# AIBluefisher/DAGSfM

Measured on AMD Instinct MI355X. Metric: verified image-pairs/sec (+ RANSAC hypotheses/sec) at 4096 feats/image, higher is better.
Workload: dtype u8 matching (int8 MFMA) + f64 verification

## Files before the change

### dagsfm_amd/capi.py

```python
import ctypes
import os

import numpy as np

_HERE = os.path.dirname(os.path.abspath(__file__))
LIB_PATH = os.environ.get("DSM_LIB_PATH") or os.path.join(_HERE, "libdagsfm_mi355x.so")
CHECK_LIB_PATH = os.environ.get("DSM_CHECK_LIB_PATH") or os.path.join(_HERE, "libdagsfm_mi355x_check.so")

GATHER_LIB_PATH = os.path.join(_HERE, "libdagsfm_gather.so")

u8p = ctypes.POINTER(ctypes.c_uint8)
u32p = ctypes.POINTER(ctypes.c_uint32)
u64p = ctypes.POINTER(ctypes.c_uint64)
f32p = ctypes.POINTER(ctypes.c_float)


class DsmError(RuntimeError):
    pass


class MatchOptions(ctypes.Structure):
    _fields_ = [("max_ratio", ctypes.c_double), ("max_distance", ctypes.c_double),
                ("cross_check", ctypes.c_int32), ("max_num_matches", ctypes.c_int32)]

# ... 1007 lines not shown
            "track_offsets": np.concatenate([[0], np.cumsum([len(t) for t in tracks])]).astype(np.uint32),
            "obs_image": np.array([img_new[int(oimg[k])] for t in tracks for k in t], np.uint32),
            "obs_xy": (np.concatenate([oxy[t] for t in tracks]) if tracks else np.zeros((0, 2))).reshape(-1, 2),
            "image_index": np.array(images, np.int64), "camera_index": np.array(cams, np.int64),
            "point_index": np.array(points, np.int64)}


def absolute_pose_seed(problem, factor_index, user_seed=0):
    return int(lib().dsm_absolute_pose_seed(problem, factor_index, user_seed))


def absolute_pose_factors(options=None):
    o = options if options is not None else default_absolute_pose_options()
    n = int(lib().dsm_absolute_pose_factors(ctypes.byref(o), None, 0))
    out = np.zeros(max(n, 1))
    lib().dsm_absolute_pose_factors(ctypes.byref(o), out.ctypes.data, n)
    return out[:n].copy()


def absolute_pose_max_trials(options=None):
    o = options if options is not None else default_absolute_pose_options()
    return int(lib().dsm_absolute_pose_max_trials(ctypes.byref(o)))


def align_seed(i, j, direction, user_seed=0):
    return int(lib().dsm_align_seed(i, j, direction, user_seed))


PRODUCT_OPTION_KEYS = ("DSM_MATCH_CHUNK_ROWS", "DSM_VERIFY_CHUNK_PAIRS", "DSM_VERIFY_LANES", "DSM_VERIFY_INLINE_LO", "DSM_VERIFY_ITEM_MODE",
                       "DSM_LO_TAIL", "DSM_LO_TAIL_MODE", "DSM_VERIFY_GRID_DIV")
CHECK_OPTION_KEYS = ("DSM_K1_DOT4", "DSM_K1_RESOLVE_KERNEL", "DSM_VERIFY_DEBUG", "DSM_SAMPLER_SERIAL", "DSM_LO_PREPARE_WAVE", "DSM_LO_JACOBI_GROUPS", "DSM_ROOTS_LDS",
                     "DSM_FINAL_WAVES", "DSM_VERIFY_LEGACY", "DSM_VERIFY_FIXED_BATCH", "DSM_VERIFY_LANE_SPLIT", "DSM_DEBUG_SAMPLER_MODE",
                     "DSM_VOCAB_ASSIGN_VALU", "DSM_VERIFY_HOST_LOOP", "DSM_SCORE_PREFILTER", "DSM_VERIFY_REPLAY_GRID", "DSM_REPLAY_LEGACY", "DSM_FLANN_GROUP", "DSM_FLANN_STATS", "DSM_ELU_LDS", "DSM_HYP_GRID", "DSM_SPEC_MARGIN",
                     "DSM_POSE_FULL", "DSM_PATCH_MATCH_LANES", "DSM_NORMS_EXACT", "DSM_FUSION_SERIAL")
DEBUG_OPTION_KEYS = PRODUCT_OPTION_KEYS


def check_requested():
    return os.environ.get("DSM_LIBRARY") == "check" or any(os.environ.get(k) is not None for k in CHECK_OPTION_KEYS)


class Context:

    def __init__(self, device=0, check=None):
        self._handle = ctypes.c_void_p()
        self._debug = {}
        self.check = check_requested() if check is None else bool(check)
        self._L = lib(self.check)
        rc = self._L.dsm_ctx_create(device, ctypes.byref(self._handle))
        if rc != 0:
            raise DsmError("dsm_ctx_create failed (%d): %s" % (rc, self._L.dsm_last_error(None).decode()))
        self.n_pairs = 0

    @property
    def _h(self):
        if self._handle:
            for key in PRODUCT_OPTION_KEYS + CHECK_OPTION_KEYS:
                want = os.environ.get(key)
                if self._debug.get(key) != want:
                    self.set_debug_option(key, want)
        return self._handle

    def set_memory_budget(self, nbytes):
        self._L.dsm_ctx_set_memory_budget.argtypes = [ctypes.c_void_p, ctypes.c_uint64]
        self._chk(self._L.dsm_ctx_set_memory_budget(self._handle, ctypes.c_uint64(int(nbytes))))

    def memory_footprint(self):
# ... 1087 lines not shown
```

### dagsfm_amd/csrc/capi.hip

```cpp
#include <hip/hip_runtime.h>
#include <math.h>
#include <stdint.h>
#include <stdio.h>
#include <stdlib.h>
#include <string.h>

#include <algorithm>
#include <string>
#include <system_error>
#include <thread>
#include <vector>

#include "../../include/dagsfm_mi355x.h"
#include "ctx.h"
#include "kernels.h"
#include "verify_camera.h"

namespace {
thread_local std::string g_create_error;
}

static const uint64_t kStageSlot = 16ull << 20;
static const uint64_t kStageSmall = 1ull << 20;
static const unsigned kStageThreads = 8;
// ... 1073 lines not shown
  vp.samples = nullptr;
  vp.draws_end = nullptr;
  vp.nmodels = nullptr;
  vp.counts = nullptr;
  vp.sums = nullptr;
  vp.first_batch[0] = vp.first_batch[1] = vp.first_batch[2] = 0;
  vp.stats = ctx->dbg("DSM_VERIFY_DEBUG") ? 1 : 0;
  vp.norms_exact = ctx->dbg("DSM_NORMS_EXACT") ? 1 : 0;
  vp.lo_reg_prepare = ctx->dbg("DSM_LO_PREPARE_WAVE") ? 0 : 1;
  vp.rp_cap = std::min<uint32_t>(n_max, 256u);
  vp.spec_margin[0] = 8;
  vp.spec_margin[1] = vp.spec_margin[2] = 4;
  if (const char* e = ctx->dbg("DSM_SPEC_MARGIN")) {
    unsigned a = 8, b = 4;
    if (sscanf(e, "%u,%u", &a, &b) == 2) {
      vp.spec_margin[0] = a;
      vp.spec_margin[1] = b;
    }
  }
  vp.hyp_map = nullptr;
  vp.hyp_seg_cap = 0;
  vp.replay_legacy = ctx->dbg("DSM_REPLAY_LEGACY") ? 1 : 0;
  vp.dbg_elu_lds = ctx->dbg("DSM_ELU_LDS") ? 1 : 0;
  vp.dbg_jacobi_groups = ctx->dbg("DSM_LO_JACOBI_GROUPS") ? 1 : 0;
  vp.dbg_roots_lds = ctx->dbg("DSM_ROOTS_LDS") ? 1 : 0;
  vp.dbg_final_waves = ctx->dbg("DSM_FINAL_WAVES") ? atoi(ctx->dbg("DSM_FINAL_WAVES")) : 0;
  vp.dbg_pose_full = ctx->dbg("DSM_POSE_FULL") ? 1 : 0;
  vp.score_prefilter = ctx->dbg("DSM_SCORE_PREFILTER") ? atoi(ctx->dbg("DSM_SCORE_PREFILTER")) : 1;
  const bool prefilter_check = ctx->dbg("DSM_SCORE_PREFILTER") && strcmp(ctx->dbg("DSM_SCORE_PREFILTER"), "check") == 0;
  if (prefilter_check) {
    vp.score_prefilter = 5;
    vp.stats = 1;
  }
  vp.models = nullptr;
  vp.e_work = nullptr;
  vp.sidx_g = nullptr;
  vp.active_count = nullptr;
  vp.lo_inl = nullptr;
  vp.worklist = nullptr;
  vp.n_work = 0;
  vp.lo_queue_g = nullptr;
  vp.lo_queue = nullptr;
  vp.lo_count = nullptr;
  vp.lo_work = vp.lo_models = vp.lo_slots = vp.lo_ework = nullptr;
  vp.tail_items = nullptr;
  vp.tail_n = nullptr;
  vp.lo_jobs = nullptr;
  vp.lo_inl_pool = nullptr;
  vp.job_list = nullptr;
#ifdef DSM_CHECK_BUILD
  const bool legacy = ctx->dbg("DSM_VERIFY_LEGACY") != nullptr;
#else
  const bool legacy = false;
#endif
  if (legacy) {
#ifdef DSM_CHECK_BUILD
    HIPCHK(ctx, ctx->d_vscratch.reserve(std::max<size_t>(1, (size_t)n_blocks * verify_scratch_bytes_per_block(n_max))));
    vp.scratch = ctx->d_vscratch.as<double>();
    HIPCHK(ctx, ctx->lanes[0].active.reserve(LANE_CTR_BYTES));
    HIPCHK(ctx, hipMemsetAsync(ctx->lanes[0].active.p, 0, LANE_CTR_BYTES, st));
    vp.active_count = ctx->lanes[0].active.as<uint32_t>() + LANE_CTR_AREA / 4;
    HIPCHK(ctx, hipEventRecord(ctx->vev0, st));
    launch_verify(vp, n_blocks, st);
    HIPCHK(ctx, hipGetLastError());
#endif
  } else {
// ... 771 lines not shown
```

### dagsfm_amd/csrc/ctx.h

```cpp
#ifndef DAGSFM_AMD_CSRC_CTX_H_
#define DAGSFM_AMD_CSRC_CTX_H_

#include <hip/hip_runtime.h>
#include <stdint.h>

#include <map>
#include <string>
#include <vector>

#include "../../include/dagsfm_mi355x.h"

struct DevBuf {
  void* p = nullptr;
  size_t cap = 0;
  DevBuf() = default;
  DevBuf(const DevBuf&) = delete;
  DevBuf& operator=(const DevBuf&) = delete;
  DevBuf(DevBuf&& o) noexcept : p(o.p), cap(o.cap) {
    o.p = nullptr;
    o.cap = 0;
  }
  DevBuf& operator=(DevBuf&& o) noexcept {
    if (this != &o) {
      release();
// ... 198 lines not shown
  std::vector<double> cluster_ritz, cluster_vectors;
  uint32_t cluster_rows = 0, cluster_cols = 0;

  template <typename F>
  void for_each_buffer(F f) {
    for (DevBuf* b : {&d_desc, &d_rterm, &d_kp, &d_img_row0, &d_img_rows, &d_lut, &d_stage, &d_counts, &d_offsets, &d_matches, &d_total, &d_etotal,
                      &d_cams, &d_pairs_dev, &d_seeds, &d_tvg, &d_inl, &d_inl_counts, &d_inl_off, &d_inl_compact, &d_inl_total, &d_nt_table,
                      &d_nt_off, &d_nt_off_t, &d_pair_state, &d_pts_px, &d_pts_norm, &d_reports, &d_masks, &d_fam_state, &d_sidx, &d_lo_inl,
                      &d_nt_table_t, &d_wm_redo, &d_wm_total, &d_wm_count, &d_lo_inl_pool, &d_pose_jobs,
                      &d_g_nfeat, &d_g_dpairs, &d_g_doff, &d_g_pdir, &d_g_params, &d_g_m, &d_g_counts, &d_g_offsets, &d_g_total, &d_g_matches,
                      &d_g_plan, &d_g_inl, &d_g_inl_off,
                      &d_mm_matches[0], &d_mm_matches[1], &d_mm_off[0], &d_mm_off[1], &d_mm_counts, &d_mm_state, &d_mm_first, &d_mm_acc,
                      &d_mm_keep, &d_mm_total, &d_vb_desc, &d_vb_idx})
      f(*b, false);
    for (DevBuf* b : {&d_m, &d_ms, &d_entries, &d_out2, &d_out2s, &d_dpairs, &d_dpairs2, &d_doutoff, &d_pair_dir, &d_order, &d_ecnt, &d_eoff,
                      &d_runs, &d_run_blocks, &d_run_blkoff, &d_gblocks, &d_egrow,
                      &d_vscratch, &d_ud_border, &d_ud_points, &d_ud_src, &d_ud_dst, &d_ud_map, &d_pm, &d_vb_point, &d_vb_node, &d_vb_embed, &d_sf_maps, &d_sf_lanes})
      f(*b, true);
    for (VerifyLane& L : lanes) L.for_each_buffer([&f](DevBuf& b) { f(b, true); });
  }
};
void dsm_retrieval_destroy(dsm_ctx* ctx);
void dsm_retrieval_invalidate(dsm_ctx* ctx);
void dsm_sift_destroy(dsm_ctx* ctx);
void dsm_covariant_sift_destroy(dsm_ctx* ctx);

static const char* const dsm_product_debug_keys[] = {"DSM_MATCH_CHUNK_ROWS", "DSM_VERIFY_CHUNK_PAIRS", "DSM_VERIFY_LANES", "DSM_VERIFY_INLINE_LO",
                                                     "DSM_VERIFY_ITEM_MODE", "DSM_LO_TAIL", "DSM_LO_TAIL_MODE", "DSM_VERIFY_GRID_DIV"};
#ifdef DSM_CHECK_BUILD
static const char* const dsm_check_debug_keys[] = {"DSM_K1_DOT4", "DSM_K1_RESOLVE_KERNEL", "DSM_VERIFY_DEBUG", "DSM_SAMPLER_SERIAL", "DSM_LO_PREPARE_WAVE", "DSM_LO_JACOBI_GROUPS",
                                                   "DSM_ROOTS_LDS", "DSM_FINAL_WAVES", "DSM_VERIFY_LEGACY", "DSM_VERIFY_FIXED_BATCH", "DSM_VERIFY_LANE_SPLIT",
                                                   "DSM_DEBUG_SAMPLER_MODE", "DSM_VOCAB_ASSIGN_VALU", "DSM_VERIFY_HOST_LOOP", "DSM_SCORE_PREFILTER",
                                                   "DSM_VERIFY_REPLAY_GRID", "DSM_REPLAY_LEGACY", "DSM_FLANN_GROUP", "DSM_FLANN_STATS", "DSM_ELU_LDS", "DSM_HYP_GRID", "DSM_SPEC_MARGIN",
                                                   "DSM_POSE_FULL", "DSM_PATCH_MATCH_LANES", "DSM_NORMS_EXACT", "DSM_FUSION_SERIAL"};
#endif

#define HIPCHK(ctx, call)                                                              \
  do {                                                                                 \
    hipError_t e_ = (call);                                                            \
    if (e_ != hipSuccess) {                                                            \
      (ctx)->err = std::string(#call) + ": " + hipGetErrorString(e_);                  \
      return DSM_ERR_HIP;                                                              \
    }                                                                                  \
  } while (0)

#define HIPTRY(call)                                                   \
  do {                                                                 \
    hipError_t e_ = (call);                                            \
    if (e_ != hipSuccess && rc == DSM_OK) {                            \
      ctx->err = std::string(#call) + ": " + hipGetErrorString(e_);    \
      rc = DSM_ERR_HIP;                                                \
    }                                                                  \
  } while (0)

static inline int dsm_fail(dsm_ctx* ctx, int code, const char* msg) {
  if (ctx) ctx->err = msg;
  return code;
}

#endif
```

### dagsfm_amd/csrc/kernels.h

```cpp
#ifndef DAGSFM_AMD_CSRC_KERNELS_H_
#define DAGSFM_AMD_CSRC_KERNELS_H_

#include <hip/hip_runtime.h>
#include <stdint.h>

#include "../../include/dagsfm_mi355x.h"

struct K1Params {
  const int8_t* desc;
  const int32_t* rterm;
  const uint2* dpairs;
  const uint32_t* img_row0;
  const uint32_t* img_rows;
  const uint64_t* d_out_off;
  const float* lut;
  float max_ratio;
  float max_distance;
  int32_t* out;
  int32_t* out_s;
  const uint32_t* order;
  const uint2* entries;
  const uint64_t* e_off;
  const uint32_t* e_cnt;
  const uint4* gblocks;
// ... 60 lines not shown
  uint32_t m_pos;
  uint32_t lo_wait;
  uint32_t lo_ninl;
  uint32_t lo_nm;
  uint32_t pad;
};
#define LO_WORK_DOUBLES 176

#define TAIL_KMAX 8
struct PoseJob {
  int32_t ncmb;
  int32_t ni;
  double Rc[4 * 9];
  double tc[4 * 3];
  int32_t cnt[4];
  double med[4];
};
struct LoJob {
  uint32_t pl;
  uint32_t ninl;
  uint32_t pending;
  uint32_t nm;
};
struct TailItem {
  uint32_t t, m;
  uint32_t nlo;
  uint32_t out_n;
  double out_sum;
  double out_model[9];
};

#ifndef DSM_REPLAY_WAVES
#define DSM_REPLAY_WAVES 4
#endif

struct VerifyParams {
  const uint32_t* pairs;
  const uint64_t* match_off;
  const uint32_t* matches;
  const double* kp;
  const uint32_t* img_row0;
  const dsm_camera* cams;
  dsm_two_view_options opt;
  const uint32_t* seeds;
  const uint32_t* nt_table;
  const uint64_t* nt_off;
  const uint32_t* nt_table_t;
  const uint64_t* nt_off_t;
  uint32_t* wm_redo;
  uint32_t* wm_total;
  uint32_t* wm_count;
  const uint32_t* final_list;
  PoseJob* pose_jobs;
  uint32_t n_final;
  uint32_t max_trials[4];
  uint32_t first_batch[3];
  dsm_two_view_geometry* tvg;
  uint32_t* inlier_matches;
  uint32_t* inl_counts;
  double* scratch;
  uint32_t* pair_state;
  double* pts_px;
  double* pts_norm;
  RansacReport* reports;
  unsigned char* masks;
  uint64_t mask_stride;
// ... 12 lines not shown
  int norms_exact;
  uint32_t spec_margin[3];
  uint32_t* hyp_map;
  uint32_t hyp_seg_cap;
  uint32_t rp_cap;
  int replay_legacy;
  double* models;
  uint32_t* sidx_g;
  uint32_t* active_count;
  uint32_t pair0, n_chunk;
  uint32_t batch;
  uint32_t n_pairs;
  uint32_t n_max;
  int32_t stage_filter;
  double* e_work;
  int32_t sampler_serial;
  int32_t reseed;
  int32_t keep_generator;
  uint32_t* lo_inl;
  TailItem* tail_items;
  uint32_t* tail_n;
  struct LoJob* lo_jobs;
  uint32_t* lo_inl_pool;
  uint32_t* job_list;
  const uint32_t* worklist;
  uint32_t n_work;
  uint32_t* lo_queue_g;
  uint32_t* lo_queue;
  uint32_t* lo_count;
  double* lo_work;
  double* lo_models;
  double* lo_slots;
  double* lo_ework;
};

size_t verify_scratch_bytes_per_block(uint32_t n_max);
size_t verify_smem_bytes(uint32_t n_max);
void launch_verify(const VerifyParams& p, uint32_t n_blocks, hipStream_t st);
void launch_vp_prep(const VerifyParams& p, uint32_t n_blocks, hipStream_t st);
void launch_vp_sample(const VerifyParams& p, int fam, uint32_t n_blocks, hipStream_t st);
void launch_vp_solve_score(const VerifyParams& p, int fam, hipStream_t st);
void launch_vp_replay(const VerifyParams& p, int fam, uint32_t n_blocks, hipStream_t st);
void launch_vp_final(const VerifyParams& p, uint32_t n_blocks, hipStream_t st);
void launch_vp_replay_lo(const VerifyParams& p, int fam, uint32_t n_blocks, int mode, hipStream_t st);
void launch_vp_items_enum(const VerifyParams& p, int fam, hipStream_t st);
void launch_vp_items_inliers(const VerifyParams& p, int fam, uint32_t n_blocks, hipStream_t st);
void launch_vp_items_outcome(const VerifyParams& p, int fam, uint32_t n_blocks, hipStream_t st);
void launch_vp_local_opt(const VerifyParams& p, int fam, uint32_t n_blocks, uint32_t n_wave_prepare, uint32_t n_small_jacobi, uint32_t n_big_prepare, hipStream_t st);
void launch_lane_counters(const void* src, uint32_t* dst_host, uint32_t copy_bytes, void* zero, size_t zero_bytes, hipStream_t st);
uint32_t vp_batch(int fam, uint32_t max_trials, uint32_t min_trials);
uint32_t vp_maxm(int fam);
void debug_read_prof(unsigned long long* out16);
void launch_debug_samples(uint32_t seed, uint32_t k, uint32_t total, uint32_t n_draws, uint32_t* out, uint32_t* idx, uint32_t* tmp7,
                          int mode, hipStream_t st);
void launch_debug_image_to_world(const dsm_camera& cam, uint32_t n, const double* xy, double* uv, hipStream_t st);
void launch_compact_inliers(const uint64_t* match_off, const uint64_t* inl_off, const uint32_t* inl_counts,
                            const uint32_t* src, uint32_t* dst, uint32_t n_pairs, hipStream_t st);

void launch_k0(const uint8_t* in_u8, int8_t* out_s8, int32_t* rterm, uint64_t n_rows, hipStream_t st);
void launch_k1(const K1Params& p, uint32_t n_directed, uint32_t max_row_blocks, hipStream_t st);
void launch_run_blocks(const uint32_t* run_first, uint32_t n_runs, const uint64_t* e_off, uint32_t* run_blocks, uint64_t* run_blkoff,
                       hipStream_t st);
void launch_gather_blocks(const uint32_t* run_first, uint32_t n_runs, const uint64_t* e_off, const uint2* dpairs, const uint64_t* run_blkoff,
                          uint4* gblocks, uint32_t n_slots, hipStream_t st);
void launch_k1_gather(const K1Params& p, uint32_t n_slots, hipStream_t st);
void launch_k1_dot4(const K1Params& p, uint32_t n_directed, uint32_t max_row_blocks, hipStream_t st);
// ... 41 lines not shown
```

### dagsfm_amd/csrc/verify_kernels.hip

```cpp
#include <hip/hip_runtime.h>
#include <stddef.h>
#include <stdint.h>

#include "../../include/dagsfm_mi355x.h"
#include "kernels.h"
#include "verify_estimators.h"
#include "verify_camera.h"
#include "verify_fivept_coop.h"

#define BATCH 64

struct MtState {
  uint32_t mt[624];
  int mti;
  uint32_t calls;
};

struct VSmem {
  WvSvdShared svd;
  double sv[9];
  double lo_models[90];
  double cur_model[9];
  double bcast[16];
  int ibcast[8];
// ... 2039 lines not shown
  for (int k = 0; k < 9; ++k) M[k] = has_model ? gm[k] : 0.0;
  int lb = 0, sure_out = n + 1;
  if (in_lds) {
    double mx[4];
    stage_points_with_maxima(gpts, n, true, spts, lane, mx);
    if (has_model) {
      const PreBounds b = prescore_bounds<FAM>(M, mx, T);
      sure_out = 0;
#pragma unroll 4
      for (int i = 0; i < n; ++i) prescore_point<FAM>(M, b, spts + (size_t)i * 4, lb, sure_out);
    }
  } else {
    double mx[4];
    stage_points_with_maxima(gpts, n, false, nullptr, lane, mx);
    if (has_model) {
      const PreBounds b = prescore_bounds<FAM>(M, mx, T);
      sure_out = 0;
#pragma unroll 4
      for (int i = 0; i < n; ++i) prescore_point<FAM>(M, b, gpts + (size_t)i * 4, lb, sure_out);
    }
  }
  if (has_slot) {
    p.counts[((size_t)pl * p.batch + t) * F::MAXM + m] = n - sure_out;
    reinterpret_cast<int32_t*>(p.sums + ((size_t)pl * p.batch + t) * F::MAXM + m)[0] = lb;
  }
}

typedef float dsm_f32x2 __attribute__((ext_vector_type(2)));
DSM_DEV dsm_f32x2 pk_fma(dsm_f32x2 a, dsm_f32x2 b, dsm_f32x2 c) { return __builtin_elementwise_fma(a, b, c); }
DSM_DEV dsm_f32x2 pk2(float x) {
  dsm_f32x2 v = {x, x};
  return v;
}
#define PRESCORE_LIST_CAP 24
__global__ __launch_bounds__(64, 6) void k_prescore_h2(const VerifyParams p) {
  extern __shared__ __attribute__((aligned(16))) unsigned char smem_raw[];
  float* s32 = reinterpret_cast<float*>(smem_raw);
  const uint32_t pl = blockIdx.x;
  const uint32_t pi = p.pair0 + pl;
  const FamState* fs = p.fam_state + (size_t)pi * 3 + FAM_H;
  if (!fs->active) return;
  const int lane = threadIdx.x;
  const int nb = (int)fs->nb;
  const int t = blockIdx.y * 64 + lane;
  if ((int)(blockIdx.y * 64) >= nb) return;
  const uint64_t moff = p.match_off[pi];
  const int n = (int)(p.match_off[pi + 1] - moff);
  const double* gpts = p.pts_px + 4 * moff;
  const bool in_lds = n <= VP_LDS_PTS;
  const double T = p.opt.max_error * p.opt.max_error;
  const bool has_slot = t < nb;
  const bool has_model = has_slot && 0 < p.nmodels[(size_t)pl * p.batch + (has_slot ? t : 0)];
  const double* gm = p.models + ((size_t)pl * p.batch + (has_slot ? t : 0)) * 9;
  double M[9];
  for (int k = 0; k < 9; ++k) M[k] = has_model ? gm[k] : 0.0;
  int lb = 0, sure_out = n + 1;
  double mx[4];
  stage_points_with_maxima(gpts, n, false, nullptr, lane, mx);
  if (!in_lds) {
    if (has_model) {
      const PreBounds b = prescore_bounds<FAM_H>(M, mx, T);
      sure_out = 0;
#pragma unroll 4
      for (int i = 0; i < n; ++i) prescore_point<FAM_H>(M, b, gpts + (size_t)i * 4, lb, sure_out);
    }
  } else {
    const int npair = (n + 1) / 2;
    uint16_t* lst = reinterpret_cast<uint16_t*>(s32 + (size_t)8 * npair);
    for (int j = lane; j < npair; j += 64) {
      const int ia = 2 * j, ib = 2 * j + 1 < n ? 2 * j + 1 : 2 * j;
      float4 lo, hi;
      lo.x = (float)gpts[ia * 4 + 0];
      lo.y = (float)gpts[ib * 4 + 0];
      lo.z = (float)gpts[ia * 4 + 1];
      lo.w = (float)gpts[ib * 4 + 1];
      hi.x = (float)gpts[ia * 4 + 2];
      hi.y = (float)gpts[ib * 4 + 2];
      hi.z = (float)gpts[ia * 4 + 3];
      hi.w = (float)gpts[ib * 4 + 3];
      reinterpret_cast<float4*>(s32)[2 * j] = lo;
      reinterpret_cast<float4*>(s32)[2 * j + 1] = hi;
    }
// ... 55 lines not shown
    }
    const bool overflow = cnt > PRESCORE_LIST_CAP;
    if (overflow) {
      lb = 0;
      sure_out = 0;
      for (int i = 0; i < n; ++i) prescore_point<FAM_H>(M, b, gpts + (size_t)i * 4, lb, sure_out);
      cnt = 0;
    }
    int maxc = cnt;
#pragma unroll
    for (int o = 32; o > 0; o >>= 1) maxc = max(maxc, __shfl_xor(maxc, o));
    for (int k0 = 0; k0 < maxc; k0 += 4) {
      double q[4][4];
      bool on[4];
#pragma unroll
      for (int u = 0; u < 4; ++u) {
        on[u] = k0 + u < cnt;
        const double* src = gpts + (size_t)(on[u] ? lst[(k0 + u) * 64 + lane] : 0) * 4;
#pragma unroll
        for (int c = 0; c < 4; ++c) q[u][c] = src[c];
      }
#pragma unroll
      for (int u = 0; u < 4; ++u) {
        bool in, out;
        prescore_flags<FAM_H>(M, b, q[u], in, out);
        lb += (on[u] && in) ? 1 : 0;
        sure_out += (on[u] && out) ? 1 : 0;
      }
    }
  }
  if (has_slot) {
    p.counts[(size_t)pl * p.batch + t] = n - sure_out;
    reinterpret_cast<int32_t*>(p.sums + (size_t)pl * p.batch + t)[0] = lb;
  }
}

#ifdef DSM_CHECK_BUILD
#define PRESCORE_CU_MFMA 0x1p-50
typedef double dsm_f64x4 __attribute__((ext_vector_type(4)));
__global__ __launch_bounds__(64, 4) void k_prescore_h_mfma(const VerifyParams p) {
  extern __shared__ __attribute__((aligned(16))) unsigned char smem_raw[];
  double* spts = reinterpret_cast<double*>(smem_raw);
  const uint32_t pl = blockIdx.x;
  const uint32_t pi = p.pair0 + pl;
  const FamState* fs = p.fam_state + (size_t)pi * 3 + FAM_H;
  if (!fs->active) return;
  const int lane = threadIdx.x;
  const int nb = (int)fs->nb;
  const int t0 = (int)blockIdx.y * 64;
  if (t0 >= nb) return;
  const uint64_t moff = p.match_off[pi];
  const int n = (int)(p.match_off[pi + 1] - moff);
  const double* gpts = p.pts_px + 4 * moff;
  const bool in_lds = n <= VP_LDS_PTS;
  const double T = p.opt.max_error * p.opt.max_error;
  const int32_t* nmod = p.nmodels + (size_t)pl * p.batch;
  const double* gmod = p.models + (size_t)pl * p.batch * 9;
  int32_t* counts = p.counts + (size_t)pl * p.batch;
  double* sums = p.sums + (size_t)pl * p.batch;
  const int t = t0 + lane;
  const bool has_slot = t < nb;
  const bool has_model = has_slot && nmod[has_slot ? t : 0] > 0;
  double M[9];
  for (int k = 0; k < 9; ++k) M[k] = has_model ? gmod[(size_t)t * 9 + k] : 0.0;
  double mx[4];
  stage_points_with_maxima(gpts, n, in_lds, spts, lane, mx);
// ... 101 lines not shown
    const int nb = (int)fs->nb;
    const uint64_t moff = p.match_off[pi];
    const int n = (int)(p.match_off[pi + 1] - moff);
    const double* gpts = (FAM == FAM_E ? p.pts_norm : p.pts_px) + 4 * moff;
    const bool in_lds = n <= VP_LDS_PTS;
    uint16_t* list = reinterpret_cast<uint16_t*>(spts + (size_t)(in_lds ? n : 0) * 4);
    __syncthreads();
    if (in_lds) (void)stage_points_batched<true, false>(gpts, 4 * n, spts, lane);
    int32_t* counts = p.counts + (size_t)pl * p.batch * F::MAXM;
    double* sums = p.sums + (size_t)pl * p.batch * F::MAXM;
    const int32_t* nmod = p.nmodels + (size_t)pl * p.batch;
    const int n_slots = nb * F::MAXM;
    int carry = (int)fs->rep.num_inliers;
    int n_list = 0;
    for (int base = 0; base < n_slots; base += 64) {
      const int slot = base + lane;
      const bool in_range = slot < n_slots;
      int ub = in_range ? counts[slot] : -1;
      if (F::MAXM > 1 && in_range && (slot % F::MAXM) >= nmod[slot / F::MAXM]) ub = -1;
      const int lb = (in_range && ub >= 0) ? reinterpret_cast<const int32_t*>(sums + slot)[0] : 0;
      int incl = lb;
#pragma unroll
      for (int o = 1; o < 64; o <<= 1) {
        const int v = __shfl_up(incl, o);
        if (lane >= o) incl = max(incl, v);
      }
      int excl = __shfl_up(incl, 1);
      if (lane == 0) excl = 0;
      const int before = max(carry, excl);
      const bool skippable = ub >= 0 && ub < before;
      const bool check = (p.score_prefilter & 4) != 0;
      if (check && skippable) atomicAdd(p.active_count + 15, 1u);
      const bool needed = ub >= 0 && (ub >= before || check);
      const unsigned long long mask = __ballot(needed);
      if (needed) list[n_list + __popcll(mask & ((1ull << lane) - 1ull))] = (uint16_t)slot;
      if (in_range && ub >= 0 && !needed) {
        counts[slot] = 0;
        sums[slot] = 0.0;
      }
      n_list += __popcll(mask);
      carry = max(carry, __shfl(incl, 63));
    }
    __syncthreads();
    double max_residual = p.opt.max_error * p.opt.max_error;
    if (FAM == FAM_E) {
      const double max_error = (image_to_world_threshold(p.cams[p.pairs[2 * pi]], p.opt.max_error) +
                                image_to_world_threshold(p.cams[p.pairs[2 * pi + 1]], p.opt.max_error)) / 2;
      max_residual = max_error * max_error;
    }
    int done = 0;
    for (; n_list - done >= 48; done += 64) {
      if (done + lane < n_list) {
        const int slot = list[done + lane];
        const double* gm = p.models + (size_t)pl * p.batch * F::MAXM * 9 + (size_t)slot * 9;
        double M[9];
        for (int k = 0; k < 9; ++k) M[k] = gm[k];
        int cnt;
        double sum;
        exact_support<FAM>(M, n, in_lds, spts, gpts, max_residual, cnt, sum);
        if (p.score_prefilter & 4) {
          const int ub = counts[slot], lb = reinterpret_cast<const int32_t*>(sums + slot)[0];
          if (cnt < lb || cnt > ub) atomicAdd(p.active_count + 14, 1u);
        }
        counts[slot] = cnt;
        sums[slot] = sum;
      }
    }
    for (int base = done; base < n_list; base += 16) {
      const int e = base + (lane >> 2);
      const bool on = e < n_list;
      const int slot = list[on ? e : base];
      const double* gm = p.models + (size_t)pl * p.batch * F::MAXM * 9 + (size_t)slot * 9;
      double M[9];
      for (int k = 0; k < 9; ++k) M[k] = gm[k];
      int cnt;
      double sum;
      exact_support_quad<FAM>(M, n, in_lds, spts, gpts, max_residual, lane, cnt, sum);
      if (on && (lane & 3) == 0) {
        if (p.score_prefilter & 4) {
          const int ub = counts[slot], lb = reinterpret_cast<const int32_t*>(sums + slot)[0];
          if (cnt < lb || cnt > ub) atomicAdd(p.active_count + 14, 1u);
        }
        counts[slot] = cnt;
        sums[slot] = sum;
      }
    }
  }
}

#define EPOLY_EB 0
template <bool COMPACT>
DSM_DEV double* e_work_of(const VerifyParams& p, uint32_t pl, int t) {
  if (COMPACT) return p.e_work + ((size_t)pl * p.batch + (size_t)(t & ~63)) * 200 + (t & 63);
  return p.e_work + ((size_t)pl * p.batch + (size_t)blockIdx.y * 64) * 200 + threadIdx.x;
}
#define EPOLY_B 36
#define EPOLY_COEFFS 75
template <bool COMPACT>
__global__ __launch_bounds__(64, 2) void k_solve_e_build(const VerifyParams p) {
  uint32_t pl;
  int t;
  if (!hyp_of_lane<COMPACT>(p, FAM_E, pl, t)) return;
  const uint32_t pi = p.pair0 + pl;
  const double* pts = p.pts_norm + 4 * p.match_off[pi];
  const uint32_t* smp = p.samples + ((size_t)pl * p.batch + t) * 7;
  double xs[20];
  auto load_sample = [&](uint32_t z) {
#pragma unroll
    for (int i = 0; i < 5; ++i) {
      const double* q = pts + (size_t)smp[z + i] * 4;
      xs[i * 4 + 0] = q[0]; xs[i * 4 + 1] = q[1]; xs[i * 4 + 2] = q[2]; xs[i * 4 + 3] = q[3];
    }
  };
  double Eb[36];
  bool exact = true;
  if (!solver_norms_exact(p)) {
    load_sample(0);
    exact = !five_point_basis_reg<true>(xs, Eb);
// ... 2301 lines not shown
  const uint32_t nb_needed = p.n_chunk < 256u * 32u ? p.n_chunk : 256u * 32u;
  if (fam == FAM_F) {
    if (p.hyp_map)
      hipLaunchKernelGGL((k_solve<FAM_F, true>), grid_hyp, dim3(64), 0, st, p);
    else
      hipLaunchKernelGGL((k_solve<FAM_F, false>), grid, dim3(64), 0, st, p);
    const size_t smem2 = smem + (size_t)p.batch * 3 * 2;
    if (p.score_prefilter && p.batch * 3 <= 65535 && smem2 <= 64 * 1024) {
      if (p.score_prefilter & 2)
        hipLaunchKernelGGL(k_prescore<FAM_F>, dim3(p.n_chunk, (p.batch * 3 + 63) / 64), dim3(64), smem, st, p);
#ifdef DSM_CHECK_BUILD
      else if (p.score_prefilter & 32)
        hipLaunchKernelGGL(k_prescore_compact<FAM_F>, dim3(p.n_chunk, (p.batch * 3 + 63) / 64), dim3(64), smem, st, p);
#endif
      else
        hipLaunchKernelGGL(k_prescore_compact2<FAM_F>, dim3(p.n_chunk, (p.batch * 3 + 63) / 64), dim3(64), smem_c2, st, p);
      hipLaunchKernelGGL(k_score_needed<FAM_F>, dim3(nb_needed), dim3(64), smem2, st, p);
    } else {
      hipLaunchKernelGGL(k_score<FAM_F>, dim3(p.n_chunk, (p.batch * 3 + 63) / 64), dim3(64), smem, st, p);
    }
  }
  if (fam == FAM_H) {
    hipLaunchKernelGGL(k_solve<FAM_H>, grid, dim3(64), 0, st, p);
    const size_t smem2 = smem + (size_t)p.batch * 2;
    if (p.score_prefilter && p.batch <= 65535 && smem2 <= 64 * 1024) {
      const size_t smem_h2 = (size_t)(p.n_max < VP_LDS_PTS ? (p.n_max > 0 ? p.n_max : 1) : VP_LDS_PTS) * 16 + 32 + (size_t)PRESCORE_LIST_CAP * 64 * 2;
#ifdef DSM_CHECK_BUILD
      if (p.score_prefilter & 8)
        hipLaunchKernelGGL(k_prescore_h_mfma, grid, dim3(64), smem, st, p);
      else if (p.score_prefilter & 16)
        hipLaunchKernelGGL(k_prescore<FAM_H>, grid, dim3(64), smem, st, p);
      else
#endif
        hipLaunchKernelGGL(k_prescore_h2, grid, dim3(64), smem_h2, st, p);
      hipLaunchKernelGGL(k_score_needed<FAM_H>, dim3(nb_needed), dim3(64), smem2, st, p);
    } else {
      hipLaunchKernelGGL(k_score<FAM_H>, grid, dim3(64), smem, st, p);
    }
  }
}
void launch_vp_replay(const VerifyParams& p, int fam, uint32_t n_blocks, hipStream_t st) {
  if (!p.n_chunk || !n_blocks) return;
  const size_t smem = ((offsetof(VSmem, gen) + 15) / 16) * 16;
  if (fam == FAM_E) hipLaunchKernelGGL(k_replay<FAM_E>, dim3(n_blocks), dim3(64), smem, st, p);
  if (fam == FAM_F) hipLaunchKernelGGL(k_replay<FAM_F>, dim3(n_blocks), dim3(64), smem, st, p);
  if (fam == FAM_H) hipLaunchKernelGGL(k_replay<FAM_H>, dim3(n_blocks), dim3(64), smem, st, p);
}
static void launch_final_pose_finish(const VerifyParams& p, uint32_t n_blocks, hipStream_t st) {
  const uint32_t n = p.final_list ? p.n_final : p.n_chunk;
  if (!n) return;
#ifdef DSM_CHECK_BUILD
  if (p.dbg_pose_full) {
    const uint32_t items = n * 4u;
    hipLaunchKernelGGL(k_final_pose_full, dim3(items < n_blocks ? items : n_blocks), dim3(64), 0, st, p);
  } else
#endif
    hipLaunchKernelGGL(k_final_pose, dim3(n < n_blocks ? n : n_blocks), dim3(64), 0, st, p);
  hipLaunchKernelGGL(k_final_finish, dim3((n + 63) / 64), dim3(64), 0, st, p);
}
void launch_vp_final(const VerifyParams& p, uint32_t n_blocks, hipStream_t st) {
  if (!p.n_pairs || !n_blocks) return;
#ifdef DSM_CHECK_BUILD
  if (p.dbg_final_waves == 1)
    hipLaunchKernelGGL(k_verify_final<1>, dim3(n_blocks), dim3(64), verify_smem_bytes(p.n_max), st, p);
  else
#endif
    hipLaunchKernelGGL(k_verify_final<2>, dim3(n_blocks), dim3(64), verify_smem_bytes(p.n_max), st, p);
// ... 234 lines not shown
```

Before: 285,600.

## Prune homography exact scoring with running best and add optional upper-bound-only prescore

Homography exact scoring in k_score_needed now walks the candidate list in chunks and tracks the best inlier count so far. After each chunk it compacts the list, dropping hypotheses whose prescore upper bound is below that best, so fewer exact f64 support evaluations are run. Separately, a debug-tunable DSM_H_LB_TRIALS option lets most blocks skip the lower-bound prescore and run only a cheaper f32 upper-bound kernel. With default settings that option leaves the old prescore launch unchanged. The pruning adds a wave-wide reduction, a list compaction and a barrier per chunk, which may cost more than it saves when few hypotheses are pruned.

```diff
diff --git a/dagsfm_amd/capi.py b/dagsfm_amd/capi.py
--- a/dagsfm_amd/capi.py
+++ b/dagsfm_amd/capi.py
@@ -1063,7 +1063,7 @@
 CHECK_OPTION_KEYS = ("DSM_K1_DOT4", "DSM_K1_RESOLVE_KERNEL", "DSM_VERIFY_DEBUG", "DSM_SAMPLER_SERIAL", "DSM_LO_PREPARE_WAVE", "DSM_LO_JACOBI_GROUPS", "DSM_ROOTS_LDS",
                      "DSM_FINAL_WAVES", "DSM_VERIFY_LEGACY", "DSM_VERIFY_FIXED_BATCH", "DSM_VERIFY_LANE_SPLIT", "DSM_DEBUG_SAMPLER_MODE",
                      "DSM_VOCAB_ASSIGN_VALU", "DSM_VERIFY_HOST_LOOP", "DSM_SCORE_PREFILTER", "DSM_VERIFY_REPLAY_GRID", "DSM_REPLAY_LEGACY", "DSM_FLANN_GROUP", "DSM_FLANN_STATS", "DSM_ELU_LDS", "DSM_HYP_GRID", "DSM_SPEC_MARGIN",
-                     "DSM_POSE_FULL", "DSM_PATCH_MATCH_LANES", "DSM_NORMS_EXACT", "DSM_FUSION_SERIAL")
+                     "DSM_POSE_FULL", "DSM_PATCH_MATCH_LANES", "DSM_NORMS_EXACT", "DSM_FUSION_SERIAL", "DSM_H_LB_TRIALS")
 DEBUG_OPTION_KEYS = PRODUCT_OPTION_KEYS
 
 
diff --git a/dagsfm_amd/csrc/capi.hip b/dagsfm_amd/csrc/capi.hip
--- a/dagsfm_amd/csrc/capi.hip
+++ b/dagsfm_amd/csrc/capi.hip
@@ -1129,6 +1129,9 @@
     vp.score_prefilter = 5;
     vp.stats = 1;
   }
+  vp.h_lb_trials = PRESCORE_H_LB_TRIALS;
+  if (const char* e = ctx->dbg("DSM_H_LB_TRIALS")) vp.h_lb_trials = (uint32_t)std::min<long>(std::max<long>(atol(e), 0), 1l << 20);
+  vp.h_lb_trials = (vp.h_lb_trials + 63u) & ~63u;
   vp.models = nullptr;
   vp.e_work = nullptr;
   vp.sidx_g = nullptr;
diff --git a/dagsfm_amd/csrc/ctx.h b/dagsfm_amd/csrc/ctx.h
--- a/dagsfm_amd/csrc/ctx.h
+++ b/dagsfm_amd/csrc/ctx.h
@@ -254,7 +254,7 @@
                                                    "DSM_ROOTS_LDS", "DSM_FINAL_WAVES", "DSM_VERIFY_LEGACY", "DSM_VERIFY_FIXED_BATCH", "DSM_VERIFY_LANE_SPLIT",
                                                    "DSM_DEBUG_SAMPLER_MODE", "DSM_VOCAB_ASSIGN_VALU", "DSM_VERIFY_HOST_LOOP", "DSM_SCORE_PREFILTER",
                                                    "DSM_VERIFY_REPLAY_GRID", "DSM_REPLAY_LEGACY", "DSM_FLANN_GROUP", "DSM_FLANN_STATS", "DSM_ELU_LDS", "DSM_HYP_GRID", "DSM_SPEC_MARGIN",
-                                                   "DSM_POSE_FULL", "DSM_PATCH_MATCH_LANES", "DSM_NORMS_EXACT", "DSM_FUSION_SERIAL"};
+                                                   "DSM_POSE_FULL", "DSM_PATCH_MATCH_LANES", "DSM_NORMS_EXACT", "DSM_FUSION_SERIAL", "DSM_H_LB_TRIALS"};
 #endif
 
 #define HIPCHK(ctx, call)                                                              \
diff --git a/dagsfm_amd/csrc/kernels.h b/dagsfm_amd/csrc/kernels.h
--- a/dagsfm_amd/csrc/kernels.h
+++ b/dagsfm_amd/csrc/kernels.h
@@ -116,6 +116,10 @@
 
 #ifndef DSM_REPLAY_WAVES
 #define DSM_REPLAY_WAVES 4
+#endif
+
+#ifndef PRESCORE_H_LB_TRIALS
+#define PRESCORE_H_LB_TRIALS (1u << 20)
 #endif
 
 struct VerifyParams {
@@ -194,6 +198,7 @@
   double* lo_models;
   double* lo_slots;
   double* lo_ework;
+  uint32_t h_lb_trials;
 };
 
 size_t verify_scratch_bytes_per_block(uint32_t n_max);
diff --git a/dagsfm_amd/csrc/verify_kernels.hip b/dagsfm_amd/csrc/verify_kernels.hip
--- a/dagsfm_amd/csrc/verify_kernels.hip
+++ b/dagsfm_amd/csrc/verify_kernels.hip
@@ -2095,6 +2095,10 @@
   dsm_f32x2 v = {x, x};
   return v;
 }
+DSM_DEV bool prescore_h_block_is_lean(const VerifyParams& p, const FamState* fs, int n) {
+  if (n > VP_LDS_PTS || p.h_lb_trials >= p.batch) return false;
+  return fs->rep.num_inliers != 0 || blockIdx.y * 64u >= p.h_lb_trials;
+}
 #define PRESCORE_LIST_CAP 24
 __global__ __launch_bounds__(64, 6) void k_prescore_h2(const VerifyParams p) {
   extern __shared__ __attribute__((aligned(16))) unsigned char smem_raw[];
@@ -2111,6 +2115,7 @@
   const int n = (int)(p.match_off[pi + 1] - moff);
   const double* gpts = p.pts_px + 4 * moff;
   const bool in_lds = n <= VP_LDS_PTS;
+  if (prescore_h_block_is_lean(p, fs, n)) return;
   const double T = p.opt.max_error * p.opt.max_error;
   const bool has_slot = t < nb;
   const bool has_model = has_slot && 0 < p.nmodels[(size_t)pl * p.batch + (has_slot ? t : 0)];
@@ -2232,6 +2237,92 @@
   if (has_slot) {
     p.counts[(size_t)pl * p.batch + t] = n - sure_out;
     reinterpret_cast<int32_t*>(p.sums + (size_t)pl * p.batch + t)[0] = lb;
+  }
+}
+
+__global__ __launch_bounds__(64, 8) void k_prescore_h_ub(const VerifyParams p) {
+  extern __shared__ __attribute__((aligned(16))) unsigned char smem_raw[];
+  float* s32 = reinterpret_cast<float*>(smem_raw);
+  const uint32_t pl = blockIdx.x;
+  const uint32_t pi = p.pair0 + pl;
+  const FamState* fs = p.fam_state + (size_t)pi * 3 + FAM_H;
+  if (!fs->active) return;
+  const int lane = threadIdx.x;
+  const int nb = (int)fs->nb;
+  const int t = blockIdx.y * 64 + lane;
+  if ((int)(blockIdx.y * 64) >= nb) return;
+  const uint64_t moff = p.match_off[pi];
+  const int n = (int)(p.match_off[pi + 1] - moff);
+  if (!prescore_h_block_is_lean(p, fs, n)) return;
+  const double* gpts = p.pts_px + 4 * moff;
+  const double T = p.opt.max_error * p.opt.max_error;
+  const bool has_slot = t < nb;
+  const bool has_model = has_slot && 0 < p.nmodels[(size_t)pl * p.batch + (has_slot ? t : 0)];
+  const double* gm = p.models + ((size_t)pl * p.batch + (has_slot ? t : 0)) * 9;
+  double M[9];
+  for (int k = 0; k < 9; ++k) M[k] = has_model ? gm[k] : 0.0;
+  double mx[4];
+  stage_points_with_maxima(gpts, n, false, nullptr, lane, mx);
+  const int npair = (n + 1) / 2;
+  for (int j = lane; j < npair; j += 64) {
+    const int ia = 2 * j, ib = 2 * j + 1 < n ? 2 * j + 1 : 2 * j;
+    float4 lo, hi;
+    lo.x = (float)gpts[ia * 4 + 0];
+    lo.y = (float)gpts[ib * 4 + 0];
+    lo.z = (float)gpts[ia * 4 + 1];
+    lo.w = (float)gpts[ib * 4 + 1];
+    hi.x = (float)gpts[ia * 4 + 2];
+    hi.y = (float)gpts[ib * 4 + 2];
+    hi.z = (float)gpts[ia * 4 + 3];
+    hi.w = (float)gpts[ib * 4 + 3];
+    reinterpret_cast<float4*>(s32)[2 * j] = lo;
+    reinterpret_cast<float4*>(s32)[2 * j + 1] = hi;
+  }
+  __syncthreads();
+  float H[9], g = __builtin_inff(), k_out = __builtin_inff();
+  {
+    const PreBounds b = prescore_bounds<FAM_H>(M, mx, T);
+    double big = 0.0;
+    for (int k = 0; k < 9; ++k) big = fmax(big, fabs(M[k]));
+    const bool usable = has_model && (b.c0 == b.c0) && big >= 0x1p-900 && big <= 0x1p900;
+    const double sc = usable ? ldexp(1.0, -ilogb(big)) : 0.0;
+    double Ms[9];
+    for (int k = 0; k < 9; ++k) {
+      Ms[k] = M[k] * sc;
+      H[k] = (float)Ms[k];
+    }
+    const double A0 = fabs(Ms[0]) * mx[0] + fabs(Ms[1]) * mx[1] + fabs(Ms[2]);
+    const double A1 = fabs(Ms[3]) * mx[0] + fabs(Ms[4]) * mx[1] + fabs(Ms[5]);
+    const double A2 = fabs(Ms[6]) * mx[0] + fabs(Ms[7]) * mx[1] + fabs(Ms[8]);
+    const double G = 6.01 * (mx[2] + mx[3]) * A2 + 5.0 * (A0 + A1 + 2.0 * A2);
+    const double gd = fmax(fmax(0x1p-24 * (58.0 * A2 + 8.6 * G / sqrt(T)), 0x1p-16 * A2), fmax(0x1p-24 * fmax(A0, A1), 0x1p-60)) * 1.001;
+    if (usable && gd <= 0x1p100) {
+      g = (float)gd * 1.0001f;
+      k_out = (float)(1.265625 * T * (1.0 + 0x1p-8)) * 1.0001f;
+    }
+  }
+  int sure_out = 0, last_b = 0;
+  const dsm_f32x2 h0 = pk2(H[0]), h1 = pk2(H[1]), h2 = pk2(H[2]), h3 = pk2(H[3]), h4 = pk2(H[4]), h5 = pk2(H[5]), h6 = pk2(H[6]), h7 = pk2(H[7]),
+                  h8 = pk2(H[8]), ko = pk2(k_out);
+  for (int j = 0; j < npair; ++j) {
+    const float4 lo = reinterpret_cast<const float4*>(s32)[2 * j], hi = reinterpret_cast<const float4*>(s32)[2 * j + 1];
+    const dsm_f32x2 s0 = {lo.x, lo.y}, s1 = {lo.z, lo.w}, d0 = {hi.x, hi.y}, d1 = {hi.z, hi.w};
+    const dsm_f32x2 p0 = pk_fma(h0, s0, pk_fma(h1, s1, h2));
+    const dsm_f32x2 p1 = pk_fma(h3, s0, pk_fma(h4, s1, h5));
+    const dsm_f32x2 p2 = pk_fma(h6, s0, pk_fma(h7, s1, h8));
+    const dsm_f32x2 e0 = pk_fma(d0, p2, -p0);
+    const dsm_f32x2 e1 = pk_fma(d1, p2, -p1);
+    const dsm_f32x2 L = pk_fma(e0, e0, e1 * e1);
+    const dsm_f32x2 Q = p2 * p2;
+    const dsm_f32x2 QO = ko * Q;
+    const bool out_a = fabsf(p2.x) >= g && (L.x > QO.x), out_b = fabsf(p2.y) >= g && (L.y > QO.y);
+    last_b = out_b ? 1 : 0;
+    sure_out += (out_a ? 1 : 0) + last_b;
+  }
+  if (n & 1) sure_out -= last_b;
+  if (has_slot) {
+    p.counts[(size_t)pl * p.batch + t] = has_model ? n - sure_out : -1;
+    reinterpret_cast<int32_t*>(p.sums + (size_t)pl * p.batch + t)[0] = 0;
   }
 }
 
@@ -2399,6 +2490,7 @@
       const bool check = (p.score_prefilter & 4) != 0;
       if (check && skippable) atomicAdd(p.active_count + 15, 1u);
       const bool needed = ub >= 0 && (ub >= before || check);
+      if (FAM == FAM_H && check && needed) reinterpret_cast<int32_t*>(sums + slot)[1] = skippable ? 1 : 0;
       const unsigned long long mask = __ballot(needed);
       if (needed) list[n_list + __popcll(mask & ((1ull << lane) - 1ull))] = (uint16_t)slot;
       if (in_range && ub >= 0 && !needed) {
@@ -2415,14 +2507,13 @@
                                 image_to_world_threshold(p.cams[p.pairs[2 * pi + 1]], p.opt.max_error)) / 2;
       max_residual = max_error * max_error;
     }
-    int done = 0;
-    for (; n_list - done >= 48; done += 64) {
+    auto walk_wave = [&](int done) -> int {
+      int cnt = 0;
       if (done + lane < n_list) {
         const int slot = list[done + lane];
         const double* gm = p.models + (size_t)pl * p.batch * F::MAXM * 9 + (size_t)slot * 9;
         double M[9];
         for (int k = 0; k < 9; ++k) M[k] = gm[k];
-        int cnt;
         double sum;
         exact_support<FAM>(M, n, in_lds, spts, gpts, max_residual, cnt, sum);
         if (p.score_prefilter & 4) {
@@ -2432,8 +2523,9 @@
         counts[slot] = cnt;
         sums[slot] = sum;
       }
-    }
-    for (int base = done; base < n_list; base += 16) {
+      return cnt;
+    };
+    auto walk_quads = [&](int base) -> int {
       const int e = base + (lane >> 2);
       const bool on = e < n_list;
       const int slot = list[on ? e : base];
@@ -2451,6 +2543,87 @@
         counts[slot] = cnt;
         sums[slot] = sum;
       }
+      return on ? cnt : 0;
+    };
+    if (FAM != FAM_H) {
+      int done = 0;
+      for (; n_list - done >= 48; done += 64) {
+        if (done + lane < n_list) {
+          const int slot = list[done + lane];
+          const double* gm = p.models + (size_t)pl * p.batch * F::MAXM * 9 + (size_t)slot * 9;
+          double M[9];
+          for (int k = 0; k < 9; ++k) M[k] = gm[k];
+          int cnt;
+          double sum;
+          exact_support<FAM>(M, n, in_lds, spts, gpts, max_residual, cnt, sum);
+          if (p.score_prefilter & 4) {
+            const int ub = counts[slot], lb = reinterpret_cast<const int32_t*>(sums + slot)[0];
+            if (cnt < lb || cnt > ub) atomicAdd(p.active_count + 14, 1u);
+          }
+          counts[slot] = cnt;
+          sums[slot] = sum;
+        }
+      }
+      for (int base = done; base < n_list; base += 16) {
+        const int e = base + (lane >> 2);
+        const bool on = e < n_list;
+        const int slot = list[on ? e : base];
+        const double* gm = p.models + (size_t)pl * p.batch * F::MAXM * 9 + (size_t)slot * 9;
+        double M[9];
+        for (int k = 0; k < 9; ++k) M[k] = gm[k];
+        int cnt;
+        double sum;
+        exact_support_quad<FAM>(M, n, in_lds, spts, gpts, max_residual, lane, cnt, sum);
+        if (on && (lane & 3) == 0) {
+          if (p.score_prefilter & 4) {
+            const int ub = counts[slot], lb = reinterpret_cast<const int32_t*>(sums + slot)[0];
+            if (cnt < lb || cnt > ub) atomicAdd(p.active_count + 14, 1u);
+          }
+          counts[slot] = cnt;
+          sums[slot] = sum;
+        }
+      }
+    } else {
+      const bool check = (p.score_prefilter & 4) != 0;
+      int done = 0, best = 0, scored = 0;
+      while (done < n_list) {
+        int top;
+        const int from = done;
+        const bool wave_trip = n_list - done >= 48 && done > 0;
+        if (check && from + lane < min(from + (wave_trip ? 64 : 16), n_list)) {
+          const int slot = list[from + lane];
+          if (reinterpret_cast<const int32_t*>(sums + slot)[1] == 0 && counts[slot] < best) atomicAdd(p.active_count + 15, 1u);
+        }
+        if (wave_trip) {
+          top = walk_wave(done);
+          done = min(done + 64, n_list);
+        } else {
+          top = walk_quads(done);
+          done = min(done + 16, n_list);
+        }
+        scored += done - from;
+#pragma unroll
+        for (int o = 32; o > 0; o >>= 1) top = max(top, __shfl_xor(top, o));
+        if (top <= best) continue;
+        best = top;
+        if (check) continue;
+        int kept = done;
+        for (int base = done; base < n_list; base += 64) {
+          const bool on = base + lane < n_list;
+          const int slot = on ? list[base + lane] : 0;
+          const bool keep = on && counts[slot] >= best;
+          const unsigned long long mask = __ballot(keep);
+          if (keep) list[kept + __popcll(mask & ((1ull << lane) - 1ull))] = (uint16_t)slot;
+          if (on && !keep) {
+            counts[slot] = 0;
+            sums[slot] = 0.0;
+          }
+          kept += __popcll(mask);
+        }
+        n_list = kept;
+        __syncthreads();
+      }
+      if (p.stats && !check && lane == 0) atomicAdd(p.active_count + 15, (uint32_t)scored);
     }
   }
 }
@@ -4818,7 +4991,13 @@
         hipLaunchKernelGGL(k_prescore<FAM_H>, grid, dim3(64), smem, st, p);
       else
 #endif
+      if (p.h_lb_trials >= p.batch) {
         hipLaunchKernelGGL(k_prescore_h2, grid, dim3(64), smem_h2, st, p);
+      } else {
+        const dim3 grid_lb(p.n_chunk, p.n_max > VP_LDS_PTS ? grid.y : p.h_lb_trials / 64);
+        if (grid_lb.y) hipLaunchKernelGGL(k_prescore_h2, grid_lb, dim3(64), smem_h2, st, p);
+        hipLaunchKernelGGL(k_prescore_h_ub, grid, dim3(64), smem_h2 - (size_t)PRESCORE_LIST_CAP * 64 * 2, st, p);
+      }
       hipLaunchKernelGGL(k_score_needed<FAM_H>, dim3(nb_needed), dim3(64), smem2, st, p);
     } else {
       hipLaunchKernelGGL(k_score<FAM_H>, grid, dim3(64), smem, st, p);
```

Result: no change. 285,300 (-0.1%).
